# Jorgenlf/Drone-2d-custom-gym-env-for-reinforcement-learning

Hardware: AMD Instinct MI355X
Metric: env-steps/sec at 65 536 parallel envs; 1/2/4/8 MI355X scaling (higher is better)
Workload: dtype f64

## Files before the change

### drone-2d-custom-gym-env-for-reinforcement-learning_amd/csrc/d2d_device.h

```cpp
#pragma once
#include <hip/hip_runtime.h>
#include <stdint.h>

#include "../../include/drone2d.h"
#include "d2d_pmath.h"

#pragma clang diagnostic ignored "-Wbitwise-instead-of-logical"

#ifdef D2D_BSTAMP
#define BST_N (1024 * 64 * 8)
__device__ uint64_t d2d_bst[BST_N];
#define BST_ARG , uint64_t* bst = nullptr
#define BST(k, dep)                                                                                      \
    do {                                                                                                 \
        if (bst) {                                                                                       \
            uint64_t bst_v;                                                                              \
            asm volatile("s_memtime %0\n\ts_waitcnt lgkmcnt(0)" : "=s"(bst_v) : "v"(dep));            \
            bst_t[k] = bst_v;                                                                            \
        }                                                                                                \
    } while (0)
#else
#define BST_ARG
#define BST(k, dep) \
    do {       \
// ... 1025 lines not shown
    if (s.r_uniform == s.r_uniform) {
        const double r = s.r_uniform;
        double q0 = __builtin_inf(), q1 = __builtin_inf(), q2 = __builtin_inf(), q3 = __builtin_inf();
        int i0 = -1, i1 = -1, i2 = -1, i3 = -1;
        for (int i = 0; i < nc; ++i) {
            const double cx = s.cx[i], cy = s.cy[i];
            const double ax = (50.0 + x) - cx, bxx = (-50.0 + x) - cx;
            const double ay = (-5.0 + y) - cy, byy = (5.0 + y) - cy;
            const double mx = fmin(fabs(ax), fabs(bxx)), my = fmin(fabs(ay), fabs(byy));
            const double q = mx * mx + my * my;
            const bool l3 = (i3 < 0) || q < q3;
            if (__ballot(l3) == 0ull) continue;
            const bool l0 = (i0 < 0) || q < q0, l1 = (i1 < 0) || q < q1, l2 = (i2 < 0) || q < q2;
            i3 = l2 ? i2 : (l3 ? i : i3);
            i2 = l1 ? i1 : (l2 ? i : i2);
            i1 = l0 ? i0 : (l1 ? i : i1);
            i0 = l0 ? i : i0;
            q3 = min_fin(q3, max_fin(q2, q));
            q2 = min_fin(q2, max_fin(q1, q));
            q1 = min_fin(q1, max_fin(q0, q));
            q0 = min_fin(q0, q);
        }
        const double d0 = sqrt_dist(q0) - r, d1 = sqrt_dist(q1) - r, d2 = sqrt_dist(q2) - r,
                     d3 = sqrt_dist(q3) - r;
        const bool tie = ((i1 >= 0) & (d1 == d0)) | ((i2 >= 0) & (d2 == d1)) | ((i3 >= 0) & (d3 == d2)) |
                         (x != x) | (y != y);
        full = tie;
        bd0 = i0 >= 0 ? d0 : bd0;
        bd1 = i1 >= 0 ? d1 : bd1;
        bd2 = i2 >= 0 ? d2 : bd2;
        bi0 = i0;
        bi1 = i1;
        bi2 = i2;
    }
    if (full) {
        bd0 = bd1 = bd2 = __builtin_inf();
        bi0 = bi1 = bi2 = -1;
    }
    for (int i = 0; i < (full ? nc : 0); ++i) {
        const double cx = s.cx[i], cy = s.cy[i];
        const double ax = (50.0 + x) - cx, bxx = (-50.0 + x) - cx;
        const double ay = (-5.0 + y) - cy, byy = (5.0 + y) - cy;
        const double mx = fmin(fabs(ax), fabs(bxx)), my = fmin(fabs(ay), fabs(byy));
        const double q = mx * mx + my * my;
        const double d = sqrt_dist(q) - s.cr[i];
        const bool l0 = (bi0 < 0) || d < bd0, l1 = (bi1 < 0) || d < bd1, l2 = (bi2 < 0) || d < bd2;
        bd2 = l1 ? bd1 : (l2 ? d : bd2);
        bi2 = l1 ? bi1 : (l2 ? i : bi2);
        bd1 = l0 ? bd0 : (l1 ? d : bd1);
        bi1 = l0 ? bi0 : (l1 ? i : bi1);
        bd0 = l0 ? d : bd0;
        bi0 = l0 ? i : bi0;
    }
    const double diag = sqrt(W * W + H * H);
    const double bd[3] = {bd0, bd1, bd2};
    const int bi[3] = {bi0, bi1, bi2};
    double sal, cal;
    sincos_d(al, sal, cal);
#pragma unroll
    for (int jj = 0; jj < 3; ++jj) {
        const int idx = bi[jj] < 0 ? 0 : bi[jj];
        const double dy = y - s.cy[idx], dx = x - s.cx[idx];
        double sa, ca;
        rel_dir(dy, dx, sal, cal, sa, ca, [&](double& rs, double& rc) {
            const double ang = ssa(atan2_d(dy, dx) - al - PI);
            sincos_d(ang, rs, rc);
            rs = -rs;
            rc = -rc;
        });
        sa = -sa;
        ca = -ca;
        const bool have = bi[jj] >= 0;
        o[8 + 3 * jj] = have ? m1to1(bd[jj], 0.0, diag) : 1.0;
        o[9 + 3 * jj] = have ? sa : 0.0;
        o[10 + 3 * jj] = have ? ca : 0.0;
    }
}
template <class S>
__device__ __forceinline__ void sensor_obs(const d2d_cfg& cfg, const S& s, const Body& F, double o[19]) {
    sensor_vel(F, o);
    sensor_pos(cfg, s, F.px, F.py, F.a, o);
}

template <class S>
__device__ __forceinline__ void path_obs_u(const d2d_cfg& cfg, const S& s, double x, double y, double al,
                                           double u, uint32_t& flags, double o[8], int iu = -1) {
    const double W = cfg.screen_w, H = cfg.screen_h;
    double cpx, cpy, u1;
    path_eval_n(s, path_k(s), u, (iu >= 0) ? iu : u_index(s, u), cpx, cpy, u1);
    const double L = SUS(s, s.n_wps - 1);
    const double ula = (u + cfg.lookahead > L) ? L : u + cfg.lookahead;
    double lax, lay;
    path_eval(s, ula, lax, lay);
    if (fabs(lax - s.wp_last_x) < 10.0 && fabs(lay - s.wp_last_y) < 10.0) flags |= D2D_FLAG_LA_LOCK;
    const bool lock = (flags & D2D_FLAG_LA_LOCK) != 0;
    lax = lock ? s.wp_last_x : lax;
    lay = lock ? s.wp_last_y : lay;
    o[0] = m1to1(cpx, 0.0, W);
    o[1] = m1to1(cpy, 0.0, H);
    o[2] = m1to1(lax, 0.0, W);
    o[3] = m1to1(lay, 0.0, H);
    const auto ref = [&](double dx, double dy, double& rs, double& rc) {
        double sa, ca;
        sincos_d(al, sa, ca);
        const double bx = fma(ca, dx, (-sa) * dy), by = fma(sa, dx, ca * dy);
        sincos_d(ssa(atan2_d(by, bx) - al), rs, rc);
    };
    const double ldx = lax - x, ldy = lay - y, cdx = cpx - x, cdy = cpy - y;
    rel_dir(ldy, ldx, 0.0, 1.0, o[4], o[5], [&](double& rs, double& rc) { ref(ldx, ldy, rs, rc); });
    rel_dir(cdy, cdx, 0.0, 1.0, o[6], o[7], [&](double& rs, double& rc) { ref(cdx, cdy, rs, rc); });
}
template <bool LT = false, bool KN = false, class S>
__device__ __forceinline__ void path_obs(const d2d_cfg& cfg, const S& s, const BrTab* T, double x, double y,
                                         double al, uint32_t& flags, double o[8], const BtHot* hot = nullptr,
                                         double* kn = nullptr) {
    int iu = -1;
    const double u = T ? (LT ? closest_u_tab<true>(s, *T, hot, x, y, iu) : closest_u_tab<false>(s, *T, &T->hot, x, y, iu))
                       : closest_u<KN>(s, x, y, iu, kn);
    path_obs_u(cfg, s, x, y, al, u, flags, o, iu);
}

template <class S>
__device__ __forceinline__ int end_cause(const d2d_cfg& cfg, const S& s, const Body& F, bool collided, int t) {
    const double W = cfg.screen_w, H = cfg.screen_h;
    const double tdx = invm1to1(m1to1(s.wp_last_x - F.px, 0.0, W), 0.0, W);
    const double tdy = invm1to1(m1to1(s.wp_last_y - F.py, 0.0, H), 0.0, H);
    const double alpha = (F.a / PI) * PI;
    int cause = 0;
    if (collided) cause |= D2D_END_COLLISION;
    if (fabs(tdx) < cfg.reach_end_radius && fabs(tdy) < cfg.reach_end_radius) cause |= D2D_END_REACH;
    if (fabs(alpha) >= cfg.aa_angle) cause |= D2D_END_AA;
    if (t == cfg.n_steps) cause |= D2D_END_TIMEUP;
    return cause;
}
struct CAStatic {
    double d, os, oc, lpa, lca, rr;
};
template <class S>
__device__ __forceinline__ CAStatic ca_static(const d2d_cfg& cfg, const S& s, const double* o) {
    const double W = cfg.screen_w, H = cfg.screen_h;
    CAStatic C{__builtin_inf(), 0.0, 1.0, 1.0, 1.0, 0.0};
    if (s.n_circles > 0) {
        const double diag = sqrt(W * W + H * H);
        const double d = invm1to1(o[8], 0.0, diag);
        C.d = d;
        C.os = o[9];
        C.oc = o[10];
        const double Rr = cfg.danger_range, k = cfg.abs_inv_ca_min_rew;
        if (d < Rr && cfg.use_lambda) {
            const double l = (d / Rr) / 2.0;
            C.lpa = (l < 0.10) ? 0.10 : l;
            C.lca = 1.0 - C.lpa;
        }
        if (d < Rr) {
            const double rr = -(((Rr + k * Rr) / (d + k * Rr)) - 1.0);
            C.rr = (rr > 0.0) ? 0.0 : rr;
        }
    }
    return C;
}
struct RewardPos {
    double aa, coll, reach, pxd, pyd;
};
__device__ __forceinline__ RewardPos reward_pos(const d2d_cfg& cfg, const Body& F, int cause, double sin_a) {
    const double W = cfg.screen_w, H = cfg.screen_h;
    RewardPos R;
    const double alpha = (F.a / PI) * PI;
    R.pxd = invm1to1(m1to1(F.px, 0.0, W), 0.0, W);
    R.pyd = invm1to1(m1to1(F.py, 0.0, H), 0.0, H);
    R.coll = (cause & D2D_END_COLLISION) ? cfg.rew_collision : 0.0;
    R.reach = (cause & D2D_END_REACH) ? cfg.rew_reach_end : 0.0;
    double aa = 0.0;
    if (alpha > cfg.aa_band) aa = -sin_a;
    if (alpha < -cfg.aa_band) aa = sin_a;
    if (cause & D2D_END_AA) aa = cfg.rew_aa;
    R.aa = aa;
    return R;
}
struct RewardVel {
    double sv, vs, vc, cal;
};
__device__ __forceinline__ RewardVel reward_vel(const d2d_cfg& cfg, const double* o, const CAStatic& C) {
    RewardVel R;
    const double vxd = invm1to1(o[0], -VEL_MAX, VEL_MAX);
    const double vyd = invm1to1(o[1], -VEL_MAX, VEL_MAX);
    R.sv = sqrt(vxd * vxd + vyd * vyd) * cfg.pp_vel_scale;
    R.vs = o[17];
    R.vc = o[18];
    double ca = 0.0;
    if (C.d < cfg.danger_range) {
        const double A = cfg.danger_angle, k = cfg.abs_inv_ca_min_rew;
        const double adiff = fabs(atan2_d(C.os * R.vc - C.oc * R.vs, C.oc * R.vc + C.os * R.vs) * (180.0 / PI));
        double ar = -(((A + k * A) / (adiff + k * A)) - 1.0);
        ar = (ar > 0.0) ? 0.0 : ar;
        ca = C.rr + ar;
    }
    R.cal = ca * C.lca;
    return R;
}
struct RewardPath {
    double ls, lc, dist, pa;
};
__device__ __forceinline__ RewardPath reward_path(const d2d_cfg& cfg, const RewardPos& P, const CAStatic& C,
                                                  const double* po) {
    const double W = cfg.screen_w, H = cfg.screen_h;
    RewardPath Q;
    const double cpx = invm1to1(po[0], 0.0, W), cpy = invm1to1(po[1], 0.0, H);
    Q.ls = po[4];
    Q.lc = po[5];
    Q.dist = norm2(cpx - P.pxd, cpy - P.pyd);
    const double pa = -(2.0 * (clipd(Q.dist, 0.0, cfg.pa_band_edge) / cfg.pa_band_edge) - 1.0) * cfg.pa_scale;
    Q.pa = pa * C.lpa;
    return Q;
}
struct RewardSum {
    double reward, pp;
};
__device__ __forceinline__ RewardSum reward_sum(const d2d_cfg& cfg, const RewardPos& P, const RewardVel& V,
                                                const RewardPath& Q) {
    RewardSum S;
    const double cvla = Q.lc * V.vc + Q.ls * V.vs;
    S.pp = clipd(cvla * V.sv, cfg.pp_rew_min, cfg.pp_rew_max);
    S.reward = P.aa + Q.pa + S.pp + P.coll + V.cal + P.reach;
    return S;
}

template <class S>
__device__ __forceinline__ void observe(const d2d_cfg& cfg, const S& s, const BrTab* T, const Body& F,
                                        uint32_t& flags, double obs[D2D_OBS_DIM]) {
    sensor_obs(cfg, s, F, obs);
    path_obs(cfg, s, T, F.px, F.py, F.a, flags, obs + 19);
}

}
```

### drone-2d-custom-gym-env-for-reinforcement-learning_amd/csrc/d2d_kernels.h

```cpp
#pragma once
#include <type_traits>

#include "d2d_curriculum.h"
#include "d2d_device.h"
#include "d2d_layout.h"

namespace d2dk {
using namespace d2d;

constexpr int BLOCK = 256;
constexpr int K1_THREADS = 256;
constexpr size_t K1_LDS_BUDGET = 40 * 1024;
constexpr size_t K2_LDS_BUDGET = 64 * 1024;
constexpr int PRIO_W0 = 2, PRIO_W1 = 1, PRIO_W2 = 3, PRIO_W3 = 1, PRIO_W2_POST = 0;

struct StepArgs {
    int n;
    int ns;
    int n_scn;
    double* st;
    int32_t* ist;
    double* acc;
    const void* scn;
    const BrTab* brt;
    int32_t* env_scn;
    int32_t* fill_ctl;
    int fill_every;
    int fill_force;
    const int32_t* pool_base;
    int pool_n;
    d2d_cfg cfg;
    double damping_dt;
    uint64_t seed;
    const float* act;
    float* obs;
    float* rew;
    uint8_t* term;
    uint8_t* trunc;
    float* info;
    float* tobs;
    const uint8_t* mask;
    uint64_t* stamps;
    float* rc_obs;
    int32_t* rc_rfl;
    int32_t* rc_tag;
    const int32_t* lane_env;
    const int32_t* wg_scn;
    const int32_t* scn_tag;
    int64_t* clock;
    int32_t* fq;
    uint32_t* fqc;
    uint32_t fq_mask;
};

template <class S>
__device__ __forceinline__ const S* scn_tab(const StepArgs& a) { return static_cast<const S*>(a.scn); }

constexpr int RC_SLOTS = 2;
constexpr int FILL_PERIOD = 16;
constexpr int FILL_EVERY = 3;
constexpr int FILL_SPB = 64;


#ifdef D2D_STAMPS
#define STAMP(k)                                                                                       \
    do {                                                                                               \
        if (a.stamps && (threadIdx.x & 63) == 0)                                                       \
            a.stamps[(size_t)(blockIdx.x * (blockDim.x >> 6) + (threadIdx.x >> 6)) * 8 + (k)] = __builtin_amdgcn_s_memtime(); \
        if (a.stamps && (threadIdx.x & 63) == 0 && (k) == 0)                                           \
            a.stamps[(size_t)(blockIdx.x * (blockDim.x >> 6) + (threadIdx.x >> 6)) * 8 + 7] =                          \
                ((uint64_t)__builtin_amdgcn_s_getreg((3 << 11) | 20) << 32) |                          \
                (uint32_t)__builtin_amdgcn_s_getreg((31 << 11) | 4) | ((uint64_t)(wave & 3) << 36) |   \
                ((uint64_t)(uint32_t)(wg + 1) << 40);                                                  \
    } while (0)
#define D2D_FSTAMP_BASE 65536
#define FSTAMP(k)                                                                                      \
    do {                                                                                               \
        if (a.stamps && (threadIdx.x & 63) == 0)                                                       \
            a.stamps[D2D_FSTAMP_BASE + (size_t)(blockIdx.x * (blockDim.x >> 6) + (threadIdx.x >> 6)) * 8 + (k)] =      \
                __builtin_amdgcn_s_memtime();                                                          \
    } while (0)
#else
#define STAMP(k) \
    do {         \
    } while (0)
#define FSTAMP(k) \
    do {          \
    } while (0)
#endif

__device__ __forceinline__ const BrTab* brtab(const StepArgs& a, int si) { return a.brt ? a.brt + si : nullptr; }
__device__ __forceinline__ size_t rc_entry(const StepArgs& a, int i, uint32_t ep) {
    return (size_t)(ep & 1u) * (size_t)a.ns + (size_t)i;
}

template <bool LDS, int NT, class S>
__device__ __forceinline__ const S* stage_scenarios(const StepArgs& a, S* lds, int first = 0, int count = -1) {
    if (!LDS) return scn_tab<S>(a);
    if (count < 0) count = a.n_scn;
    const int words = count * (int)(sizeof(S) / 8);
    const double* src = reinterpret_cast<const double*>(scn_tab<S>(a) + first);
    double* dst = reinterpret_cast<double*>(lds);
    for (int k = threadIdx.x; k < words; k += NT) dst[k] = src[k];
    return lds - first;
}
template <int NT>
__device__ __forceinline__ const BtHot* stage_hot(const StepArgs& a, BtHot* lds, int first = 0, int count = -1) {
    if (count < 0) count = a.n_scn;
    const int per = (int)(sizeof(BtHot) / 16);
    for (int k = threadIdx.x; k < count * per; k += NT) {
        const double2* src = reinterpret_cast<const double2*>(&a.brt[first + k / per].hot) + (k % per);
        reinterpret_cast<double2*>(lds)[k] = *src;
    }
    return lds - first;
}
template <int NWAVES>
__device__ __forceinline__ void glds_copy(void* lds_dst, const void* gsrc, int bytes) {
    using LP = __attribute__((address_space(3))) void;
    using GP = __attribute__((address_space(1))) void;
    const int wave = __builtin_amdgcn_readfirstlane(threadIdx.x >> 6), lane = threadIdx.x & 63;
    for (int c = wave; c * 1024 < bytes; c += NWAVES) {
        const int off = c * 1024 + lane * 16;
        if (off < bytes)
            __builtin_amdgcn_global_load_lds((GP*)((const char*)gsrc + off), (LP*)((char*)lds_dst + c * 1024), 16, 0, 0);
    }
}

__device__ __forceinline__ size_t fidx(int f, int n, int i) { return (size_t)f * (size_t)n + (size_t)i; }
template <typename T>
__device__ __forceinline__ T& fld(T* base, int f, int n, int i) {
    T* fb = base + (size_t)__builtin_amdgcn_readfirstlane(f) * (size_t)__builtin_amdgcn_readfirstlane(n);
    return fb[i];
}

__device__ __forceinline__ Body load_frame(const StepArgs& a, int i) {
    const int n = a.ns;
    return Body{fld(a.st, 0, n, i), fld(a.st, 1, n, i), fld(a.st, 2, n, i),
                fld(a.st, 3, n, i), fld(a.st, 4, n, i), fld(a.st, 5, n, i)};
}
template <class SC>
__device__ __forceinline__ void spawn_state(const StepArgs& a, const SC& S, int i, uint32_t ep, double sp[7]) {
    double x, y, th;
    spawn_draw(S, a.seed, (uint32_t)a.cfg.env_id_base + (uint32_t)i, ep, x, y, th);
    double sl, cl, sr, cr;
    sincos_d(th + PI, sl, cl);
    sincos_d(th, sr, cr);
    sp[0] = x;
    sp[1] = y;
    sp[2] = th;
    sp[3] = cl * DRONE_R + x;
    sp[4] = sl * DRONE_R + y;
    sp[5] = cr * DRONE_R + x;
    sp[6] = sr * DRONE_R + y;
}

using LdsU32 = __attribute__((address_space(3))) uint32_t;
__device__ __forceinline__ bool flag_seen(const uint32_t& f) {
    return __builtin_amdgcn_readfirstlane(*(const volatile LdsU32*)&f) != 0u;
}
__device__ __forceinline__ int pool_scenario(const StepArgs& a, int j, uint32_t ep) {
    return *a.pool_base + (a.pool_n > 1 ? pool_pick(a.seed, (uint32_t)a.cfg.env_id_base + (uint32_t)j, ep, a.pool_n) : 0);
}
__device__ __forceinline__ int fresh_slot(int j, uint32_t ep) { return 2 * j + (int)(ep & 1u); }
enum { FR_HEAD = 0, FR_TAIL0 = 1, FR_TAIL1 = 2, FR_WORDS = 4 };
__device__ __forceinline__ int next_scenario(const StepArgs& a, int j, uint32_t ep) {
    if (a.cfg.scn_pool == 2) return fresh_slot(j, ep);
    if (a.cfg.scn_pool) return pool_scenario(a, j, ep);
    if (a.n_scn <= 1) return 0;
    return a.env_scn[j];
}

struct K1Shared {
    double cas[6][EPB];
    int scn[EPB];
    uint8_t cause[EPB];
    uint8_t cvalid[EPB];
    uint32_t pflags[EPB];
    uint32_t ep[EPB];
    double sina[EPB];
    uint32_t w0t[EPB], w0fl[EPB];
    uint32_t f_done, f_ca, f_gs, f_rp, f_ver, f_ver1, f_acc, n_tile;
    double pe[2][EPB];
    double acc[D2D_NSTATS][EPB];
    union {
        struct {
            double jb[6 * JB_PER_JOINT][EPB];
            double arms[ARMS_N][EPB];
        } g;
        struct {
            double post[7][EPB];
            alignas(16) float obs[EPB * D2D_OBS_DIM];
        } p;
    } u;
};

__device__ __forceinline__ int lane_fresh() {
    int l;
    asm volatile("v_mbcnt_lo_u32_b32 %0, -1, 0\n\tv_mbcnt_hi_u32_b32 %0, -1, %0" : "=v"(l));
    return l;
}
__device__ __forceinline__ void flag_raise(uint32_t& f) {
    __builtin_amdgcn_fence(__ATOMIC_RELEASE, "workgroup");
    if ((threadIdx.x & 63) == 0) *(volatile LdsU32*)&f = 1u;
}
__device__ __forceinline__ void flag_wait(const uint32_t& f) {
    while (!flag_seen(f)) __builtin_amdgcn_s_sleep(1)  ;
    __builtin_amdgcn_fence(__ATOMIC_ACQUIRE, "workgroup");
}
__device__ __forceinline__ void tile_arrive(uint32_t& c) {
    __builtin_amdgcn_fence(__ATOMIC_RELEASE, "workgroup");
    if ((threadIdx.x & 63) == 0) atomicAdd(&c, 1u);
}
__device__ __forceinline__ void tile_wait(const uint32_t& c, uint32_t n) {
    while (__builtin_amdgcn_readfirstlane(*(const volatile LdsU32*)&c) < n) __builtin_amdgcn_s_sleep(1);
    __builtin_amdgcn_fence(__ATOMIC_ACQUIRE, "workgroup");
}

template <bool LT, class SC>
__device__ __forceinline__ double bt_finish_join(const SC& s, const BrTab& T, const BtHot* hot, const BtLane& L,
                                                 const uint32_t& fv, const uint32_t& dv, double px, double py,
                                                 int& iu) {
    constexpr int IT_JOIN = 200;
    static_assert(BT_RIDE < IT_JOIN, "the riders' passes end below the first loop's cap");
    const PathK K = path_k(s);
    const bool early = L.dev < L.len;
    if constexpr (BT_RIDE > 0) {
        const bool rider = !early & (L.len > BT_EARLY);
        const bool any_rider = __ballot(rider) != 0ull;
        Brent B;
        bt_restore(T.snap[L.kind][rider ? BT_EARLY : L.dev], B);
        if (__ballot(early) != 0ull) {
            if (early) bt_restore_f<LT>(T.snap[L.kind][L.dev], hot, L.kind, px, py, B);
        }
        if (rider) {
            B.ffulc = L.fa;
            B.fnfc = L.fb;
            B.fx = L.fc;
        }
        const bool in = early | rider;
        uint32_t up = 0u;
        int it = 0;
        for (;; ++it) {
            const bool open = in & brent_open(B);
            const bool go = (any_rider & (it < BT_RIDE)) |
                            ((__builtin_amdgcn_readfirstlane(up) == 0u) & (__ballot(early & open) != 0ull));
            if (!(open & (it < IT_JOIN) & go)) break;
            up = *(const volatile LdsU32*)&fv;
            brent_step(s, K, px, py, B);
        }
        B.num += it;
        flag_wait(fv);
        const uint32_t m = min((uint32_t)L.len, dv);
        bool jump = false;
        if (__ballot(rider & brent_open(B)) != 0ull) {
            const int q = min(BT_EARLY + it, L.len);
            const BtSnap& Q = T.snap[L.kind][q];
            const auto same = [](double x, double y) { return __double_as_longlong(x) == __double_as_longlong(y); };
            const bool eq = same(B.a, Q.a) & same(B.b, Q.b) & same(B.fulc, Q.fulc) & same(B.nfc, Q.nfc) &
                            same(B.xf, Q.xf) & same(B.rat, Q.rat) & same(B.e, Q.e) & (B.ia == Q.ia) &
                            (B.ib == Q.ib) & (B.ixf == Q.ixf);
            jump = rider & brent_open(B) & (it >= BT_RIDE) & eq & (m >= (uint32_t)q);
        }
        const bool late = jump | (!in & ((dv < (uint32_t)L.len) | brent_active(B)));
        if (__ballot(late) != 0ull) {
            if (late) {
                const BtSnap& S = T.snap[L.kind][m];
                bt_restore(S, B);
                if (brent_active(B)) bt_restore_f<LT>(S, hot, L.kind, px, py, B);
            }
        }
        if (__ballot(brent_active(B)) != 0ull)
            brent_run(s, K, px, py, B, nullptr, 500 - (BT_K_MAX + 1) - IT_JOIN);
        iu = B.ixf;
        return B.xf;
    }
    Brent B;
    bt_restore(T.snap[L.kind][L.dev], B);
    if (__ballot(early) != 0ull) {
        if (early) bt_restore_f<LT>(T.snap[L.kind][L.dev], hot, L.kind, px, py, B);
        uint32_t up = 0u;
        int it = 0;
        for (;; ++it) {
            if (!(early & brent_open(B) & (it < IT_JOIN) & (__builtin_amdgcn_readfirstlane(up) == 0u))) break;
            up = *(const volatile LdsU32*)&fv;
            brent_step(s, K, px, py, B);
        }
        B.num += it;
    }
    flag_wait(fv);
    const bool late = !early & ((dv < (uint32_t)L.len) | brent_active(B));
    if (__ballot(late) != 0ull) {
        if (late) {
            const BtSnap& S = T.snap[L.kind][min((uint32_t)L.len, dv)];
            bt_restore(S, B);
            bt_restore_f<LT>(S, hot, L.kind, px, py, B);
        }
    }
    if (__ballot(brent_active(B)) != 0ull) brent_run(s, K, px, py, B, nullptr, 500 - (BT_K_MAX + 1) - IT_JOIN);
    iu = B.ixf;
    return B.xf;
}

template <bool LDS, bool LTAB, bool GRP, class S>
__device__ __forceinline__ void k1_stage(const StepArgs& a, S* s_scn, int wg, const S*& scns,
                                         const BtHot*& hots, int& s0) {
    const int ws = (GRP && LDS) ? a.wg_scn[wg] : 0;
    s0 = ws >= 0 ? ws : -ws - 2;
    const int ncopy = (GRP && LDS) ? (ws >= 0 ? 1 : 2) : a.n_scn;
    hots = nullptr;
    if (LDS && (ncopy == 1 || !LTAB)) {
        glds_copy<K1_THREADS / 64>(s_scn, scn_tab<S>(a) + s0, (int)sizeof(S) * ncopy);
        if (LTAB) glds_copy<K1_THREADS / 64>(s_scn + 1, &a.brt[s0].hot, (int)sizeof(BtHot));
        scns = s_scn - s0;
        if (LTAB) hots = reinterpret_cast<const BtHot*>(s_scn + 1) - s0;
    } else {
        scns = stage_scenarios<LDS, K1_THREADS>(a, s_scn, s0, ncopy);
        if (LTAB) hots = stage_hot<K1_THREADS>(a, reinterpret_cast<BtHot*>(s_scn + ncopy), s0, ncopy);
    }
}

extern __shared__ __attribute__((aligned(16))) uint4 d2d_dyn_lds[];
constexpr int K1_KN_BYTES = D2D_MAX_WPS * 64 * 8;
template <bool LDS, bool LTAB, bool GRP, bool S3, class SC>
__device__ __forceinline__ void k1_body(const StepArgs& a, const SC* scns, const BtHot* hots, int s0, K1Shared& sh,
                                        int wg, int role, int qt) {
    const int wave = role;
    const int lane = threadIdx.x & 63;
    const bool gvalid = wg >= 0;
    const int e0 = gvalid ? wg * EPB : 0;
    const int i = e0 + lane;
    const int ie = (GRP && gvalid) ? a.lane_env[i] : i;
    const bool valid = gvalid && (GRP ? ie >= 0 : i < a.n);
    const int n = a.ns;
    const bool auto_reset = a.cfg.auto_reset != 0;
    constexpr bool EARLY = LDS && LTAB && !S3 && BT_EARLY > 0 && (!GRP || D2D_BT_EARLY_GRP);
    STAMP(0);
    if (wg == 0 && qt == 0 && a.fill_ctl)
        __hip_atomic_store(&a.fill_ctl[0], __hip_atomic_load(&a.fill_ctl[1], __ATOMIC_RELAXED, __HIP_MEMORY_SCOPE_AGENT),
                           __ATOMIC_RELAXED, __HIP_MEMORY_SCOPE_AGENT);
    if (wg == 0 && qt == 0 && a.clock)
        __hip_atomic_fetch_add(a.clock, (int64_t)1, __ATOMIC_RELAXED, __HIP_MEMORY_SCOPE_AGENT);
    if (wave == 0) sh.scn[lane] = (valid && a.env_scn && a.n_scn > 1) ? a.env_scn[ie] : s0;
    if (S3 && wave == 0) sh.pflags[lane] = 0x7fffffffu;
    Body PF{};
    if (valid && wave != 0) PF = load_frame(a, i);
    if (qt == 0) {
        sh.f_done = 0u;
        sh.f_ca = 0u;
        sh.f_gs = 0u;
        sh.f_rp = 0u;
        sh.f_ver = 0u;
        sh.f_ver1 = 0u;
        sh.f_acc = 0u;
        sh.n_tile = 0u;
    }
    __syncthreads();
    STAMP(1);
    const SC& S = scns[sh.scn[lane]];
    float* const trow = a.tobs ? a.tobs + (size_t)ie * D2D_OBS_DIM : nullptr;
    float* const orow = &sh.u.p.obs[lane * D2D_OBS_DIM];

    Body F0{};
    double path_err = 0.0, tot_rew = 0.0;
    int t = 0, cause = 0;
    uint32_t flags = 0;
    RewardVel RV{};
    double dclose = 0.0, rew_sum = 0.0, rew_pp = 0.0, pdist = 0.0;
    uint32_t plal = 0;
    bool done = false;
    if (wave == 0) {
        __builtin_amdgcn_s_setprio(PRIO_W0);
        double ov[19];
        Body B[3];
        double j[12], cs[3], sn[3], fx = 0.0, fy = 0.0, tq = 0.0;
        if (valid) {
#pragma unroll
            for (int b = 0; b < 3; ++b) {
                B[b].px = fld(a.st, 6 * b + 0, n, i);
                B[b].py = fld(a.st, 6 * b + 1, n, i);
                B[b].a = fld(a.st, 6 * b + 2, n, i);
                B[b].vx = fld(a.st, 6 * b + 3, n, i);
                B[b].vy = fld(a.st, 6 * b + 4, n, i);
                B[b].w = fld(a.st, 6 * b + 5, n, i);
            }
#pragma unroll
            for (int k = 0; k < 12; ++k) j[k] = fld(a.st, D2D_S_J + k, n, i);
            t = fld(a.ist, D2D_I_T, n, i);
            flags = (uint32_t)fld(a.ist, D2D_I_FLAGS, n, i);
            const float2 act = reinterpret_cast<const float2*>(a.act)[ie];
            const float fs = (float)a.cfg.force_scale;
            const float lf = __fmul_rn(__fadd_rn(act.x / 2.0f, 0.5f), fs);
            const float rf = __fmul_rn(__fadd_rn(act.y / 2.0f, 0.5f), fs);
            if (phys_positions(S, B, (double)lf, (double)rf, cs, sn, fx, fy, tq)) flags |= D2D_FLAG_COLLIDED;
            t += 1;
            cause = end_cause(a.cfg, S, B[0], (flags & D2D_FLAG_COLLIDED) != 0, t);
            done = cause != 0;
            const int32_t ep = fld(a.ist, D2D_I_EPISODE, n, i);
            const bool cv = done && auto_reset && a.rc_tag[rc_entry(a, i, (uint32_t)ep)] == ep;
            sh.ep[lane] = (uint32_t)ep;
            sh.cause[lane] = (uint8_t)cause;
            sh.sina[lane] = sn[0];
            sh.cvalid[lane] = cv ? 1u : 0u;
            sh.w0t[lane] = (uint32_t)t;
            sh.w0fl[lane] = flags;
            if (!(done && auto_reset)) {
#pragma unroll
                for (int b = 0; b < 3; ++b) {
                    fld(a.st, 6 * b + 0, n, i) = B[b].px;
                    fld(a.st, 6 * b + 1, n, i) = B[b].py;
                    fld(a.st, 6 * b + 2, n, i) = B[b].a;
                }
            }
        }
        flag_raise(sh.f_done);
        if (valid) {
            const Arms A = make_arms(cs, sn);
            const double pos[6] = {B[0].px, B[0].py, B[1].px, B[1].py, B[2].px, B[2].py};
            double vel[9] = {B[0].vx, B[0].vy, B[0].w, B[1].vx, B[1].vy, B[1].w, B[2].vx, B[2].vy, B[2].w};
            phys_velocities<true>(A, pos, a.damping_dt, fx, fy, tq, vel, j, &sh.u.g.jb[0][lane], EPB,
                                  &sh.u.g.arms[0][lane]);
            asm volatile("" ::: "memory");
            const int ln = lane_fresh(), iw = e0 + ln;
            const uint32_t cw = sh.cause[ln];
            cause = (int)cw;
            done = cw != 0u;
            t = (int)sh.w0t[ln];
            flags = sh.w0fl[ln];
            if (!(done && auto_reset)) {
#pragma unroll
            for (int b = 0; b < 3; ++b) {
                fld(a.st, 6 * b + 3, n, iw) = vel[3 * b + 0];
                fld(a.st, 6 * b + 4, n, iw) = vel[3 * b + 1];
                fld(a.st, 6 * b + 5, n, iw) = vel[3 * b + 2];
            }
#pragma unroll
            for (int k = 0; k < 12; ++k) fld(a.st, D2D_S_J + k, n, iw) = j[k];
            }
            F0 = Body{0.0, 0.0, B[0].a, vel[0], vel[1], vel[2]};
        }
        flag_raise(sh.f_gs);
        STAMP(4);
        const int ln = lane_fresh(), iw = e0 + ln, iew = GRP ? ie : iw;
        const bool vw = gvalid && (GRP ? iew >= 0 : iw < a.n);
        if (vw) {
            float* const orw = &sh.u.p.obs[ln * D2D_OBS_DIM];
            float* const trw = a.tobs ? a.tobs + (size_t)iew * D2D_OBS_DIM : nullptr;
            sensor_vel(F0, sh.sina[ln], cs[0], ov);
            if (!(done && auto_reset)) {
                orw[0] = (float)ov[0];
                orw[1] = (float)ov[1];
                orw[2] = (float)ov[2];
                orw[17] = (float)ov[17];
                orw[18] = (float)ov[18];
            }
            if (done && trw) {
                trw[0] = (float)ov[0];
                trw[1] = (float)ov[1];
                trw[2] = (float)ov[2];
                trw[17] = (float)ov[17];
                trw[18] = (float)ov[18];
            }
        }
        tile_arrive(sh.n_tile);
        flag_wait(sh.f_ca);
        STAMP(5);
        if (vw) {
            CAStatic C;
            C.d = sh.cas[0][ln];
            C.os = sh.cas[1][ln];
            C.oc = sh.cas[2][ln];
            C.lpa = sh.cas[3][ln];
            C.lca = sh.cas[4][ln];
            C.rr = sh.cas[5][ln];
            RV = reward_vel(a.cfg, ov, C);
            dclose = C.d;
        }
        if (!S3) {
            flag_wait(sh.f_acc);
            const int lp = lane_fresh();
            path_err = sh.pe[0][lp];
            tot_rew = sh.pe[1][lp];
        }
        flag_wait(sh.f_rp);
        if (vw) {
            RewardPos RP{};
            RP.aa = sh.u.p.post[4][ln];
            RP.coll = sh.u.p.post[5][ln];
            RP.reach = sh.u.p.post[6][ln];
            RewardPath RQ{};
            RQ.ls = sh.u.p.post[0][ln];
            RQ.lc = sh.u.p.post[1][ln];
            RQ.pa = sh.u.p.post[2][ln];
            if (!GRP) {
                pdist = sh.u.p.post[3][ln];
                plal = sh.pflags[ln];
            }
            const RewardSum Q = reward_sum(a.cfg, RP, RV, RQ);
            rew_sum = Q.reward;
            rew_pp = Q.pp;
        }
    } else if (wave == 1) {
        float row[19];
        bool need = false;
        if (S3) {
            __builtin_amdgcn_s_setprio(PRIO_W2);
            if (valid && a.brt) {
                const BrTab& T = a.brt[sh.scn[lane]];
                const BtHot* hot = LTAB ? hots + sh.scn[lane] : &T.hot;
                Body F = PF;
                advance_position(F);
                BtLane L = bt_start<LTAB>(T, hot, F.px, F.py);
                const int k0 = bt_third(T, 1), k1 = bt_third(T, 2);
                if (k0 < min(k1, L.len)) {
                    if (k0 >= 4) bt_window<LTAB>(hot, L, k0, F.px, F.py);
                else bt_window_snap<LTAB>(T, hot, L, k0, F.px, F.py);
                    bt_verify<LTAB>(hot, L, k0, k1, F.px, F.py);
                }
                atomicMin(&sh.pflags[lane], (uint32_t)L.dev);
            }
            flag_raise(sh.f_ver1);
        }
        __builtin_amdgcn_s_setprio(PRIO_W1);
        if (valid) {
            Body F = PF;
            advance_position(F);
            double so[19];
            sensor_pos(a.cfg, S, F.px, F.py, F.a, so);
            const CAStatic C = ca_static(a.cfg, S, so);
            sh.cas[0][lane] = C.d;
            sh.cas[1][lane] = C.os;
            sh.cas[2][lane] = C.oc;
            sh.cas[3][lane] = C.lpa;
            sh.cas[4][lane] = C.lca;
            sh.cas[5][lane] = C.rr;
#pragma unroll
            for (int k = 0; k < 19; ++k) row[k] = (float)so[k];
        }
        flag_raise(sh.f_ca);
        flag_wait(sh.f_done);
        if (valid) {
            done = sh.cause[lane] != 0u;
            need = done && auto_reset;
            if (done && trow) {
#pragma unroll
                for (int k = 3; k < 17; ++k) trow[k] = row[k];
            }
        }
        if (__ballot(need) != 0ull) {
            if (need) {
                if (sh.cvalid[lane] != 0u) {
                    const float* c = a.rc_obs + rc_entry(a, i, sh.ep[lane]) * D2D_OBS_DIM;
#pragma unroll
                    for (int k = 0; k < 19; ++k) row[k] = c[k];
                } else {
                    const uint32_t ep = sh.ep[lane];
                    const SC& SN = scns[next_scenario(a, ie, ep)];
                    double sp[7], so[19];
                    spawn_state(a, SN, ie, ep, sp);
                    sensor_obs(a.cfg, SN, Body{sp[0], sp[1], sp[2], 0.0, 0.0, 0.0}, so);
#pragma unroll
                    for (int k = 0; k < 19; ++k) row[k] = (float)so[k];
                }
            }
        }
        STAMP(4);
        flag_wait(sh.f_gs);
        STAMP(5);
        if (valid) {
            if (need) {
#pragma unroll
                for (int k = 0; k < 19; ++k) orow[k] = row[k];
            } else {
#pragma unroll
                for (int k = 3; k < 17; ++k) orow[k] = row[k];
            }
        }
        tile_arrive(sh.n_tile);
    } else if (wave == 2) {
        __builtin_amdgcn_s_setprio(PRIO_W2);
        double po[8];
        Body F{};
        if (valid) {
            F = PF;
            advance_position(F);
            uint32_t f = (uint32_t)fld(a.ist, D2D_I_FLAGS, n, i);
            const BrTab* T = brtab(a, sh.scn[lane]);
            if (T) {
                const BtHot* hot = LTAB ? hots + sh.scn[lane] : &T->hot;
                BtLane L = bt_start<LTAB>(*T, hot, F.px, F.py);
                int iu;
                double u;
                if constexpr (EARLY) {
                    bt_verify<LTAB>(hot, L, 1, BT_EARLY, F.px, F.py);
                    u = bt_finish_join<LTAB>(S, *T, hot, L, sh.f_ver, sh.pflags[lane], F.px, F.py, iu);
                } else {
                    bt_verify<LTAB>(hot, L, 1, !LDS ? BT_K : S3 ? bt_third(*T, 1) : bt_split(*T), F.px, F.py);
                    flag_wait(sh.f_ver);
                    if (S3) flag_wait(sh.f_ver1);
                    L.dev = min(L.dev, (int)sh.pflags[lane]);
                    u = bt_finish<LTAB>(S, *T, hot, L.kind, L.dev, F.px, F.py, iu);
                }
                path_obs_u(a.cfg, S, F.px, F.py, F.a, u, f, po, iu);
            } else {
                path_obs<LTAB, SC::RM>(a.cfg, S, T, F.px, F.py, F.a, f, po, LTAB ? hots + sh.scn[lane] : nullptr,
                                       SC::RM ? reinterpret_cast<double*>(d2d_dyn_lds) : nullptr);
            }
            sh.pflags[lane] = f & D2D_FLAG_LA_LOCK;
        }
        STAMP(4);
        __builtin_amdgcn_s_setprio(PRIO_W2_POST);
        flag_wait(sh.f_done);
        flag_wait(sh.f_ca);
        RewardPos RP{};
        RewardPath RQ{};
        bool d = false;
        if (valid) {
            const int cause = (int)sh.cause[lane];
            d = cause != 0;
            CAStatic C;
            C.lpa = sh.cas[3][lane];
            RP = reward_pos(a.cfg, F, cause, sh.sina[lane]);
            RQ = reward_path(a.cfg, RP, C, po);
        }
        flag_wait(sh.f_gs);
        if (valid) {
            if (!(d && auto_reset)) {
#pragma unroll
                for (int k = 0; k < 8; ++k) orow[19 + k] = (float)po[k];
            }
            if (d && trow) {
#pragma unroll
                for (int k = 0; k < 8; ++k) trow[19 + k] = (float)po[k];
            }
        }
        if (valid) {
            sh.u.p.post[0][lane] = RQ.ls;
            sh.u.p.post[1][lane] = RQ.lc;
            sh.u.p.post[2][lane] = RQ.pa;
            sh.u.p.post[3][lane] = RQ.dist;
            sh.u.p.post[4][lane] = RP.aa;
            sh.u.p.post[5][lane] = RP.coll;
            sh.u.p.post[6][lane] = RP.reach;
        }
        flag_raise(sh.f_rp);
        tile_arrive(sh.n_tile);
        STAMP(5);
    } else {
        __builtin_amdgcn_s_setprio(PRIO_W2);
        double po[8];
        if (!LDS) {
            sh.pflags[lane] = 0x7fffffffu;
        } else if (valid && a.brt) {
            const BrTab& T = a.brt[sh.scn[lane]];
            const BtHot* hot = LTAB ? hots + sh.scn[lane] : &T.hot;
            Body F = PF;
            advance_position(F);
            BtLane L = bt_start<LTAB>(T, hot, F.px, F.py);
            const int k0 = EARLY ? BT_EARLY + BT_RIDE : S3 ? bt_third(T, 2) : bt_split(T);
            if (k0 < L.len) {
                if (k0 >= 4) bt_window<LTAB>(hot, L, k0, F.px, F.py);
                else bt_window_snap<LTAB>(T, hot, L, k0, F.px, F.py);
                bt_verify<LTAB>(hot, L, k0, BT_K, F.px, F.py);
            }
            if (S3) atomicMin(&sh.pflags[lane], (uint32_t)L.dev);
            else sh.pflags[lane] = (uint32_t)L.dev;
        }
        flag_raise(sh.f_ver);
        __builtin_amdgcn_s_setprio(PRIO_W3);
        if (valid) {
            sh.pe[0][lane] = fld(a.st, D2D_S_PATH_ERR, n, i);
            sh.pe[1][lane] = fld(a.st, D2D_S_TOT_REW, n, i);
        }
        flag_wait(sh.f_done);
        const bool cv = valid && sh.cvalid[lane] != 0u;
        if (valid) done = sh.cause[lane] != 0u;
        if (valid && done) {
#pragma unroll
            for (int k = 0; k < D2D_NSTATS; ++k) sh.acc[k][lane] = fld(a.acc, k, n, i);
        }
        flag_raise(sh.f_acc);
        if (valid && done && auto_reset) {
            const uint32_t ep = sh.ep[lane];
            const int nscn = next_scenario(a, ie, ep);
            const SC& SN = scns[nscn];
            double sp[7];
            spawn_state(a, SN, ie, ep, sp);
            uint32_t rfl = 0;
            if (cv) {
                const size_t ce = rc_entry(a, i, ep);
                const float* c = a.rc_obs + ce * D2D_OBS_DIM + 19;
#pragma unroll
                for (int k = 0; k < 8; ++k) po[k] = (double)c[k];
                rfl = (uint32_t)a.rc_rfl[ce];
            } else {
                path_obs(a.cfg, SN, brtab(a, nscn), sp[0], sp[1], sp[2], rfl, po);
            }
            const double th = sp[2];
            const double bodies[18] = {sp[0], sp[1], th, 0.0, 0.0, 0.0, sp[3], sp[4], th, 0.0, 0.0, 0.0,
                                       sp[5], sp[6], th, 0.0, 0.0, 0.0};
#pragma unroll
            for (int f = 0; f < 18; ++f) fld(a.st, f, n, i) = bodies[f];
#pragma unroll
            for (int k = 0; k < 12; ++k) fld(a.st, D2D_S_J + k, n, i) = 0.0;
            fld(a.st, D2D_S_PATH_ERR, n, i) = 0.0;
            fld(a.st, D2D_S_TOT_REW, n, i) = 0.0;
            fld(a.ist, D2D_I_T, n, i) = 0;
            fld(a.ist, D2D_I_FLAGS, n, i) = (int32_t)rfl;
            fld(a.ist, D2D_I_EPISODE, n, i) = (int32_t)(ep + 1u);
            if (a.cfg.scn_pool && a.env_scn) a.env_scn[ie] = nscn;
        }
        if (!LDS && a.fq) {
            const bool need = valid && done && auto_reset;
            const uint64_t m = __ballot(need);
            if (m != 0ull) {
                const int first = __ffsll((unsigned long long)m) - 1;
                uint32_t base = 0;
                if (lane == first) base = atomicAdd(&a.fqc[FR_HEAD], (uint32_t)__popcll(m));
                base = __shfl(base, first);
                const uint32_t pos = base + (uint32_t)__popcll(m & ((1ull << lane) - 1ull));
                if (need) a.fq[pos & a.fq_mask] = fresh_slot(ie, sh.ep[lane] + 1u);
            }
        }
        STAMP(4);
        flag_wait(sh.f_gs);
        STAMP(5);
        if (valid && done && auto_reset) {
#pragma unroll
            for (int k = 0; k < 8; ++k) orow[19 + k] = (float)po[k];
        }
        tile_arrive(sh.n_tile);
    }
    STAMP(2);

    if (wave != 0) {
        tile_wait(sh.n_tile, 4u);
        STAMP(3);
        constexpr int TT = K1_THREADS - 64;
        const int tq = qt - 64;
        if (GRP) {
            for (int k = tq; gvalid && k < EPB * D2D_OBS_DIM; k += TT) {
                const int r = k / D2D_OBS_DIM;
                const int e = a.lane_env[e0 + r];
                if (e >= 0) a.obs[(size_t)e * D2D_OBS_DIM + (k - r * D2D_OBS_DIM)] = sh.u.p.obs[k];
            }
        } else {
            const int rows = gvalid ? max(0, min(EPB, a.n - e0)) : 0;
            const int words = rows * D2D_OBS_DIM;
            float* dst = a.obs + (size_t)e0 * D2D_OBS_DIM;
            int k0 = 0;
            if (rows == EPB && ((uintptr_t)a.obs & 15u) == 0) {
                float4* d4 = reinterpret_cast<float4*>(dst);
                const float4* s4 = reinterpret_cast<const float4*>(sh.u.p.obs);
                for (int k = tq; k < words / 4; k += TT) d4[k] = s4[k];
                k0 = words;
            }
            for (int k = k0 + tq; k < words; k += TT) dst[k] = sh.u.p.obs[k];
        }
    } else {
        if (S3) flag_wait(sh.f_acc);
        STAMP(3);
    }
    const int lne = lane_fresh(), ile = e0 + lne, iee = GRP ? ie : ile;
    const bool vle = gvalid && (GRP ? iee >= 0 : ile < a.n);
    if (wave == 0 && vle) {
        const int lane = lne, i = ile, ie = iee;
        if (S3) {
            path_err = sh.pe[0][lane];
            tot_rew = sh.pe[1][lane];
        }
        flags = (flags & ~D2D_FLAG_LA_LOCK) | (GRP ? sh.pflags[lane] : plal);
        const double reward = rew_sum;
        path_err += GRP ? sh.u.p.post[3][lane] : pdist;
        const double ape_g = GRP ? path_err / (double)t : 0.0;
        tot_rew += reward;
        bool trunc = false, term = done;
        if (a.cfg.timeup_truncates && done && cause == D2D_END_TIMEUP) {
            trunc = true;
            term = false;
        }
        const int io = ie;
        a.rew[io] = (float)reward;
        a.term[io] = (uint8_t)term;
        a.trunc[io] = (uint8_t)trunc;
        if (a.info) {
            float* r = a.info + (size_t)ie * D2D_INFO_DIM;
            r[D2D_INFO_CA] = (float)RV.cal;
            r[D2D_INFO_PA] = (float)sh.u.p.post[2][lane];
            r[D2D_INFO_PP] = (float)rew_pp;
            r[D2D_INFO_COLL] = (float)sh.u.p.post[5][lane];
            r[D2D_INFO_REACH] = (float)sh.u.p.post[6][lane];
            r[D2D_INFO_AA] = (float)sh.u.p.post[4][lane];
            r[D2D_INFO_DCLOSE] = (float)dclose;
            r[D2D_INFO_STEPS] = (float)t;
            r[D2D_INFO_CAUSE] = (float)cause;
            r[D2D_INFO_APE] = done ? (float)(GRP ? ape_g : path_err / (double)t) : 0.0f;
            r[D2D_INFO_TOTREW] = done ? (float)tot_rew : 0.0f;
            r[D2D_INFO_REWARD] = (float)reward;
        }
        if (done) {
            double pacc[D2D_NSTATS];
#pragma unroll
            for (int k = 0; k < D2D_NSTATS; ++k) pacc[k] = sh.acc[k][lane];
            const double ape = GRP ? ape_g : path_err / (double)t;
            const bool c1 = cause & D2D_END_COLLISION, c2 = cause & D2D_END_REACH;
            const bool c4 = cause & D2D_END_TIMEUP, c5 = cause & D2D_END_AA;
            fld(a.acc, D2D_ST_RETURN, n, i) = pacc[D2D_ST_RETURN] + tot_rew;
            fld(a.acc, D2D_ST_EPISODES, n, i) = pacc[D2D_ST_EPISODES] + 1.0;
            fld(a.acc, D2D_ST_SUCCESS, n, i) = pacc[D2D_ST_SUCCESS] + (c2 ? 1.0 : 0.0);
            fld(a.acc, D2D_ST_FAIL, n, i) = pacc[D2D_ST_FAIL] + ((c1 || c4 || c5) ? 1.0 : 0.0);
            fld(a.acc, D2D_ST_COLLISION, n, i) = pacc[D2D_ST_COLLISION] + ((c1 && !c2 && !c4 && !c5) ? 1.0 : 0.0);
            fld(a.acc, D2D_ST_APE, n, i) = pacc[D2D_ST_APE] + ape;
// ... 373 lines not shown
```

Measured before the change: 2.559 billion.

## Split path-observation tail across waves and poll three flags in one LDS read

Adds an optional mode, off by default (D2D_TAIL_SPLIT=0), that splits the path observation into a closest-point part and a lookahead part. Another wave that has parked can take the lookahead evaluation and its reward terms, coordinated through a new bitmask flag in LDS. Separately, it enables by default a single 16-byte LDS read that checks three completion flags at once, so the common case skips three sequential spin-waits. The split adds cross-wave handshakes and code complexity. The combined flag check saves only a few LDS polls.

```diff
diff --git a/drone-2d-custom-gym-env-for-reinforcement-learning_amd/csrc/d2d_device.h b/drone-2d-custom-gym-env-for-reinforcement-learning_amd/csrc/d2d_device.h
--- a/drone-2d-custom-gym-env-for-reinforcement-learning_amd/csrc/d2d_device.h
+++ b/drone-2d-custom-gym-env-for-reinforcement-learning_amd/csrc/d2d_device.h
@@ -1131,33 +1131,63 @@
     sensor_pos(cfg, s, F.px, F.py, F.a, o);
 }
 
-template <class S>
-__device__ __forceinline__ void path_obs_u(const d2d_cfg& cfg, const S& s, double x, double y, double al,
-                                           double u, uint32_t& flags, double o[8], int iu = -1) {
+template <bool CP, bool LA, class S>
+__device__ __forceinline__ void path_obs_parts(const d2d_cfg& cfg, const S& s, double x, double y, double al,
+                                               double u, uint32_t& flags, double o[8], int iu) {
     const double W = cfg.screen_w, H = cfg.screen_h;
     double cpx, cpy, u1;
-    path_eval_n(s, path_k(s), u, (iu >= 0) ? iu : u_index(s, u), cpx, cpy, u1);
-    const double L = SUS(s, s.n_wps - 1);
-    const double ula = (u + cfg.lookahead > L) ? L : u + cfg.lookahead;
+    if constexpr (CP) path_eval_n(s, path_k(s), u, (iu >= 0) ? iu : u_index(s, u), cpx, cpy, u1);
     double lax, lay;
-    path_eval(s, ula, lax, lay);
-    if (fabs(lax - s.wp_last_x) < 10.0 && fabs(lay - s.wp_last_y) < 10.0) flags |= D2D_FLAG_LA_LOCK;
-    const bool lock = (flags & D2D_FLAG_LA_LOCK) != 0;
-    lax = lock ? s.wp_last_x : lax;
-    lay = lock ? s.wp_last_y : lay;
-    o[0] = m1to1(cpx, 0.0, W);
-    o[1] = m1to1(cpy, 0.0, H);
-    o[2] = m1to1(lax, 0.0, W);
-    o[3] = m1to1(lay, 0.0, H);
+    if constexpr (LA) {
+        const double L = SUS(s, s.n_wps - 1);
+        const double ula = (u + cfg.lookahead > L) ? L : u + cfg.lookahead;
+        path_eval(s, ula, lax, lay);
+        if (fabs(lax - s.wp_last_x) < 10.0 && fabs(lay - s.wp_last_y) < 10.0) flags |= D2D_FLAG_LA_LOCK;
+        const bool lock = (flags & D2D_FLAG_LA_LOCK) != 0;
+        lax = lock ? s.wp_last_x : lax;
+        lay = lock ? s.wp_last_y : lay;
+    }
+    if constexpr (CP) {
+        o[0] = m1to1(cpx, 0.0, W);
+        o[1] = m1to1(cpy, 0.0, H);
+    }
+    if constexpr (LA) {
+        o[2] = m1to1(lax, 0.0, W);
+        o[3] = m1to1(lay, 0.0, H);
+    }
     const auto ref = [&](double dx, double dy, double& rs, double& rc) {
         double sa, ca;
         sincos_d(al, sa, ca);
         const double bx = fma(ca, dx, (-sa) * dy), by = fma(sa, dx, ca * dy);
         sincos_d(ssa(atan2_d(by, bx) - al), rs, rc);
     };
-    const double ldx = lax - x, ldy = lay - y, cdx = cpx - x, cdy = cpy - y;
-    rel_dir(ldy, ldx, 0.0, 1.0, o[4], o[5], [&](double& rs, double& rc) { ref(ldx, ldy, rs, rc); });
-    rel_dir(cdy, cdx, 0.0, 1.0, o[6], o[7], [&](double& rs, double& rc) { ref(cdx, cdy, rs, rc); });
+    double ldx, ldy, cdx, cdy;
+    if constexpr (LA) {
+        ldx = lax - x;
+        ldy = lay - y;
+    }
+    if constexpr (CP) {
+        cdx = cpx - x;
+        cdy = cpy - y;
+    }
+    if constexpr (LA) rel_dir(ldy, ldx, 0.0, 1.0, o[4], o[5], [&](double& rs, double& rc) { ref(ldx, ldy, rs, rc); });
+    if constexpr (CP) rel_dir(cdy, cdx, 0.0, 1.0, o[6], o[7], [&](double& rs, double& rc) { ref(cdx, cdy, rs, rc); });
+}
+template <class S>
+__device__ __forceinline__ void path_obs_cp(const d2d_cfg& cfg, const S& s, double x, double y, double al,
+                                            double u, int iu, double o[8]) {
+    uint32_t none = 0;
+    path_obs_parts<true, false>(cfg, s, x, y, al, u, none, o, iu);
+}
+template <class S>
+__device__ __forceinline__ void path_obs_la(const d2d_cfg& cfg, const S& s, double x, double y, double al,
+                                            double u, uint32_t& flags, double o[8]) {
+    path_obs_parts<false, true>(cfg, s, x, y, al, u, flags, o, -1);
+}
+template <class S>
+__device__ __forceinline__ void path_obs_u(const d2d_cfg& cfg, const S& s, double x, double y, double al,
+                                           double u, uint32_t& flags, double o[8], int iu = -1) {
+    path_obs_parts<true, true>(cfg, s, x, y, al, u, flags, o, iu);
 }
 template <bool LT = false, bool KN = false, class S>
 __device__ __forceinline__ void path_obs(const d2d_cfg& cfg, const S& s, const BrTab* T, double x, double y,
@@ -1250,13 +1280,14 @@
 struct RewardPath {
     double ls, lc, dist, pa;
 };
+template <bool LA = true>
 __device__ __forceinline__ RewardPath reward_path(const d2d_cfg& cfg, const RewardPos& P, const CAStatic& C,
                                                   const double* po) {
     const double W = cfg.screen_w, H = cfg.screen_h;
     RewardPath Q;
     const double cpx = invm1to1(po[0], 0.0, W), cpy = invm1to1(po[1], 0.0, H);
-    Q.ls = po[4];
-    Q.lc = po[5];
+    Q.ls = LA ? po[4] : 0.0;
+    Q.lc = LA ? po[5] : 0.0;
     Q.dist = norm2(cpx - P.pxd, cpy - P.pyd);
     const double pa = -(2.0 * (clipd(Q.dist, 0.0, cfg.pa_band_edge) / cfg.pa_band_edge) - 1.0) * cfg.pa_scale;
     Q.pa = pa * C.lpa;
diff --git a/drone-2d-custom-gym-env-for-reinforcement-learning_amd/csrc/d2d_kernels.h b/drone-2d-custom-gym-env-for-reinforcement-learning_amd/csrc/d2d_kernels.h
--- a/drone-2d-custom-gym-env-for-reinforcement-learning_amd/csrc/d2d_kernels.h
+++ b/drone-2d-custom-gym-env-for-reinforcement-learning_amd/csrc/d2d_kernels.h
@@ -13,6 +13,12 @@
 constexpr size_t K1_LDS_BUDGET = 40 * 1024;
 constexpr size_t K2_LDS_BUDGET = 64 * 1024;
 constexpr int PRIO_W0 = 2, PRIO_W1 = 1, PRIO_W2 = 3, PRIO_W3 = 1, PRIO_W2_POST = 0;
+#ifndef D2D_TAIL_SPLIT
+#define D2D_TAIL_SPLIT 0
+#endif
+#ifndef D2D_TAIL_WAIT3
+#define D2D_TAIL_WAIT3 1
+#endif
 
 struct StepArgs {
     int n;
@@ -73,6 +79,11 @@
                 (uint32_t)__builtin_amdgcn_s_getreg((31 << 11) | 4) | ((uint64_t)(wave & 3) << 36) |   \
                 ((uint64_t)(uint32_t)(wg + 1) << 40);                                                  \
     } while (0)
+#define STAMP_ROUTE(s)                                                                                 \
+    do {                                                                                               \
+        if (a.stamps && (threadIdx.x & 63) == 0 && (s))                                                \
+            a.stamps[(size_t)(blockIdx.x * (blockDim.x >> 6) + (threadIdx.x >> 6)) * 8 + 7] |= 1ull << 38; \
+    } while (0)
 #define D2D_FSTAMP_BASE 65536
 #define FSTAMP(k)                                                                                      \
     do {                                                                                               \
@@ -83,6 +94,9 @@
 #else
 #define STAMP(k) \
     do {         \
+    } while (0)
+#define STAMP_ROUTE(s) \
+    do {               \
     } while (0)
 #define FSTAMP(k) \
     do {          \
@@ -170,6 +184,7 @@
     return a.env_scn[j];
 }
 
+enum : uint32_t { TL_PARK = 1u, TL_TAKE = 2u, TL_KEEP = 4u, TL_LA = 8u };
 struct K1Shared {
     double cas[6][EPB];
     int scn[EPB];
@@ -207,6 +222,31 @@
     while (!flag_seen(f)) __builtin_amdgcn_s_sleep(1)  ;
     __builtin_amdgcn_fence(__ATOMIC_ACQUIRE, "workgroup");
 }
+__device__ __forceinline__ bool flags3_seen(const K1Shared& sh) {
+    static_assert(offsetof(K1Shared, f_done) % 16 == 0 && offsetof(K1Shared, f_ca) == offsetof(K1Shared, f_done) + 4 &&
+                      offsetof(K1Shared, f_gs) == offsetof(K1Shared, f_done) + 8,
+                  "one 16-byte read");
+    typedef uint32_t u32x4 __attribute__((ext_vector_type(4)));
+    using LdsU32x4 = __attribute__((address_space(3))) u32x4;
+    const u32x4 v = *(const volatile LdsU32x4*)&sh.f_done;
+    const bool up = (__builtin_amdgcn_readfirstlane(v.x) != 0u) & (__builtin_amdgcn_readfirstlane(v.y) != 0u) &
+                    (__builtin_amdgcn_readfirstlane(v.z) != 0u);
+    if (up) __builtin_amdgcn_fence(__ATOMIC_ACQUIRE, "workgroup");
+    return up;
+}
+__device__ __forceinline__ void bits_raise(uint32_t& f, uint32_t bits) {
+    __builtin_amdgcn_fence(__ATOMIC_RELEASE, "workgroup");
+    if ((threadIdx.x & 63) == 0) atomicOr(&f, bits);
+}
+__device__ __forceinline__ uint32_t bits_seen(const uint32_t& f) {
+    return __builtin_amdgcn_readfirstlane(*(const volatile LdsU32*)&f);
+}
+__device__ __forceinline__ uint32_t bits_wait(const uint32_t& f, uint32_t mask) {
+    uint32_t v;
+    while (((v = bits_seen(f)) & mask) == 0u) __builtin_amdgcn_s_sleep(1);
+    __builtin_amdgcn_fence(__ATOMIC_ACQUIRE, "workgroup");
+    return v;
+}
 __device__ __forceinline__ void tile_arrive(uint32_t& c) {
     __builtin_amdgcn_fence(__ATOMIC_RELEASE, "workgroup");
     if ((threadIdx.x & 63) == 0) atomicAdd(&c, 1u);
@@ -334,6 +374,9 @@
     const int n = a.ns;
     const bool auto_reset = a.cfg.auto_reset != 0;
     constexpr bool EARLY = LDS && LTAB && !S3 && BT_EARLY > 0 && (!GRP || D2D_BT_EARLY_GRP);
+    constexpr bool TAIL = EARLY && D2D_TAIL_SPLIT;
+    constexpr bool WAIT3 = EARLY && D2D_TAIL_WAIT3;
+    uint32_t& f_tail = sh.f_ver1;
     STAMP(0);
     if (wg == 0 && qt == 0 && a.fill_ctl)
         __hip_atomic_store(&a.fill_ctl[0], __hip_atomic_load(&a.fill_ctl[1], __ATOMIC_RELAXED, __HIP_MEMORY_SCOPE_AGENT),
@@ -482,6 +525,7 @@
             tot_rew = sh.pe[1][lp];
         }
         flag_wait(sh.f_rp);
+        if constexpr (TAIL) bits_wait(f_tail, TL_LA);
         if (vw) {
             RewardPos RP{};
             RP.aa = sh.u.p.post[4][ln];
@@ -580,16 +624,17 @@
         __builtin_amdgcn_s_setprio(PRIO_W2);
         double po[8];
         Body F{};
+        double u = 0.0;
+        int iu = -1;
+        uint32_t f = 0;
         if (valid) {
             F = PF;
             advance_position(F);
-            uint32_t f = (uint32_t)fld(a.ist, D2D_I_FLAGS, n, i);
+            f = (uint32_t)fld(a.ist, D2D_I_FLAGS, n, i);
             const BrTab* T = brtab(a, sh.scn[lane]);
             if (T) {
                 const BtHot* hot = LTAB ? hots + sh.scn[lane] : &T->hot;
                 BtLane L = bt_start<LTAB>(*T, hot, F.px, F.py);
-                int iu;
-                double u;
                 if constexpr (EARLY) {
                     bt_verify<LTAB>(hot, L, 1, BT_EARLY, F.px, F.py);
                     u = bt_finish_join<LTAB>(S, *T, hot, L, sh.f_ver, sh.pflags[lane], F.px, F.py, iu);
@@ -600,17 +645,43 @@
                     L.dev = min(L.dev, (int)sh.pflags[lane]);
                     u = bt_finish<LTAB>(S, *T, hot, L.kind, L.dev, F.px, F.py, iu);
                 }
-                path_obs_u(a.cfg, S, F.px, F.py, F.a, u, f, po, iu);
+                if constexpr (!TAIL) path_obs_u(a.cfg, S, F.px, F.py, F.a, u, f, po, iu);
             } else {
-                path_obs<LTAB, SC::RM>(a.cfg, S, T, F.px, F.py, F.a, f, po, LTAB ? hots + sh.scn[lane] : nullptr,
-                                       SC::RM ? reinterpret_cast<double*>(d2d_dyn_lds) : nullptr);
-            }
-            sh.pflags[lane] = f & D2D_FLAG_LA_LOCK;
-        }
-        STAMP(4);
+                if constexpr (!TAIL)
+                    path_obs<LTAB, SC::RM>(a.cfg, S, T, F.px, F.py, F.a, f, po, LTAB ? hots + sh.scn[lane] : nullptr,
+                                           SC::RM ? reinterpret_cast<double*>(d2d_dyn_lds) : nullptr);
+                else
+                    u = closest_u<false>(S, F.px, F.py, iu, nullptr);
+            }
+            if constexpr (!TAIL) sh.pflags[lane] = f & D2D_FLAG_LA_LOCK;
+        }
+        bool split = false;
+        if constexpr (TAIL) {
+            STAMP(4);
+            split = (bits_seen(f_tail) & TL_PARK) != 0u;
+            STAMP_ROUTE(split);
+            if (split) {
+                __builtin_amdgcn_fence(__ATOMIC_ACQUIRE, "workgroup");
+                if (valid) sh.acc[D2D_ST_PAD][lane] = u;
+                bits_raise(f_tail, TL_TAKE);
+                if (valid) path_obs_cp(a.cfg, S, F.px, F.py, F.a, u, iu, po);
+            } else {
+                bits_raise(f_tail, TL_KEEP);
+                if (valid) {
+                    path_obs_u(a.cfg, S, F.px, F.py, F.a, u, f, po, iu);
+                    sh.pflags[lane] = f & D2D_FLAG_LA_LOCK;
+                }
+            }
+        } else {
+            STAMP(4);
+        }
         __builtin_amdgcn_s_setprio(PRIO_W2_POST);
-        flag_wait(sh.f_done);
-        flag_wait(sh.f_ca);
+        bool up3 = false;
+        if constexpr (WAIT3) up3 = flags3_seen(sh);
+        if (!up3) {
+            flag_wait(sh.f_done);
+            flag_wait(sh.f_ca);
+        }
         RewardPos RP{};
         RewardPath RQ{};
         bool d = false;
@@ -620,27 +691,47 @@
             CAStatic C;
             C.lpa = sh.cas[3][lane];
             RP = reward_pos(a.cfg, F, cause, sh.sina[lane]);
-            RQ = reward_path(a.cfg, RP, C, po);
-        }
-        flag_wait(sh.f_gs);
-        if (valid) {
-            if (!(d && auto_reset)) {
-#pragma unroll
-                for (int k = 0; k < 8; ++k) orow[19 + k] = (float)po[k];
-            }
-            if (d && trow) {
-#pragma unroll
-                for (int k = 0; k < 8; ++k) trow[19 + k] = (float)po[k];
-            }
-        }
-        if (valid) {
-            sh.u.p.post[0][lane] = RQ.ls;
-            sh.u.p.post[1][lane] = RQ.lc;
-            sh.u.p.post[2][lane] = RQ.pa;
-            sh.u.p.post[3][lane] = RQ.dist;
-            sh.u.p.post[4][lane] = RP.aa;
-            sh.u.p.post[5][lane] = RP.coll;
-            sh.u.p.post[6][lane] = RP.reach;
+            if (split) RQ = reward_path<false>(a.cfg, RP, C, po);
+            else RQ = reward_path(a.cfg, RP, C, po);
+        }
+        if (!up3) flag_wait(sh.f_gs);
+        if (split) {
+            if (valid) {
+                if (!(d && auto_reset)) {
+                    orow[19] = (float)po[0];
+                    orow[20] = (float)po[1];
+                    orow[25] = (float)po[6];
+                    orow[26] = (float)po[7];
+                }
+                if (d && trow) {
+                    trow[19] = (float)po[0];
+                    trow[20] = (float)po[1];
+                    trow[25] = (float)po[6];
+                    trow[26] = (float)po[7];
+                }
+                sh.u.p.post[2][lane] = RQ.pa;
+                sh.u.p.post[3][lane] = RQ.dist;
+            }
+        } else {
+            if (valid) {
+                if (!(d && auto_reset)) {
+#pragma unroll
+                    for (int k = 0; k < 8; ++k) orow[19 + k] = (float)po[k];
+                }
+                if (d && trow) {
+#pragma unroll
+                    for (int k = 0; k < 8; ++k) trow[19 + k] = (float)po[k];
+                }
+            }
+            if (valid) {
+                sh.u.p.post[0][lane] = RQ.ls;
+                sh.u.p.post[1][lane] = RQ.lc;
+                sh.u.p.post[2][lane] = RQ.pa;
+                sh.u.p.post[3][lane] = RQ.dist;
+                sh.u.p.post[4][lane] = RP.aa;
+                sh.u.p.post[5][lane] = RP.coll;
+                sh.u.p.post[6][lane] = RP.reach;
+            }
         }
         flag_raise(sh.f_rp);
         tile_arrive(sh.n_tile);
@@ -671,6 +762,10 @@
             sh.pe[0][lane] = fld(a.st, D2D_S_PATH_ERR, n, i);
             sh.pe[1][lane] = fld(a.st, D2D_S_TOT_REW, n, i);
         }
+        uint32_t lfl = 0;
+        if constexpr (TAIL) {
+            if (valid) lfl = (uint32_t)fld(a.ist, D2D_I_FLAGS, n, i);
+        }
         flag_wait(sh.f_done);
         const bool cv = valid && sh.cvalid[lane] != 0u;
         if (valid) done = sh.cause[lane] != 0u;
@@ -679,6 +774,15 @@
             for (int k = 0; k < D2D_NSTATS; ++k) sh.acc[k][lane] = fld(a.acc, k, n, i);
         }
         flag_raise(sh.f_acc);
+        Body FL{};
+        RewardPos RL{};
+        if constexpr (TAIL) {
+            if (valid) {
+                FL = PF;
+                advance_position(FL);
+                RL = reward_pos(a.cfg, FL, (int)sh.cause[lane], sh.sina[lane]);
+            }
+        }
         if (valid && done && auto_reset) {
             const uint32_t ep = sh.ep[lane];
             const int nscn = next_scenario(a, ie, ep);
@@ -722,11 +826,37 @@
             }
         }
         STAMP(4);
+        bool took = false;
+        double lo[8];
+        if constexpr (TAIL) {
+            bits_raise(f_tail, TL_PARK);
+            took = (bits_wait(f_tail, TL_TAKE | TL_KEEP) & TL_TAKE) != 0u;
+            if (took && valid) path_obs_la(a.cfg, S, FL.px, FL.py, FL.a, sh.acc[D2D_ST_PAD][lane], lfl, lo);
+        }
         flag_wait(sh.f_gs);
         STAMP(5);
         if (valid && done && auto_reset) {
 #pragma unroll
             for (int k = 0; k < 8; ++k) orow[19 + k] = (float)po[k];
+        }
+        if constexpr (TAIL) {
+            if (took && valid) {
+                if (!(done && auto_reset)) {
+#pragma unroll
+                    for (int k = 2; k < 6; ++k) orow[19 + k] = (float)lo[k];
+                }
+                if (done && trow) {
+#pragma unroll
+                    for (int k = 2; k < 6; ++k) trow[19 + k] = (float)lo[k];
+                }
+                sh.u.p.post[0][lane] = lo[4];
+                sh.u.p.post[1][lane] = lo[5];
+                sh.u.p.post[4][lane] = RL.aa;
+                sh.u.p.post[5][lane] = RL.coll;
+                sh.u.p.post[6][lane] = RL.reach;
+                sh.pflags[lane] = lfl & D2D_FLAG_LA_LOCK;
+            }
+            bits_raise(f_tail, TL_LA);
         }
         tile_arrive(sh.n_tile);
     }
```

New measurement: 2.573 billion (median of 6 runs). No clear change (+0.6%).
